# AssemblyAI-Community/MinImagen

Hardware: AMD Instinct MI355X
Metric: denoising-steps/sec (images/sec x T), base 64^2 + SR 64->256 cascade (higher is better)
Workload: dtype f32; 1 GPU; cascade64_256: unet_0 params @64x64 + unet_1 params (lowres_cond) @256x256, T=100/stage, cond_scale=3.0 (2 U-Net evals/step), dynamic thresholding 0.9, fp32 storage / accumulate / softmax / statistics, contractions as 3-term fp16-split (hi*hi + hi*lo + lo*hi) MFMA products; per_gpu_batch=32, global_batch=32, parallelism=dp1

## Files before the change

include/minimagen_hip.h:

```cpp
#ifndef MINIMAGEN_HIP_H
#define MINIMAGEN_HIP_H

#include <stdint.h>

#ifdef __cplusplus
extern "C" {
#endif

#define MI_ABI_VERSION 12

enum mi_status {
    MI_OK = 0,
    MI_ERR_INVALID = -1,
    MI_ERR_LAUNCH = -2,
    MI_ERR_UNSUPPORTED = -3
};

int mi_abi_version(void);
const char* mi_last_error(void);
const char* mi_backend(void);
int mi_struct_size(int which);

typedef struct mi_act {
    const float* data;
// ... 46 lines not shown
int mi_conv_fwd(const mi_conv_params* p, void* stream);
int mi_gn_coef_fwd(const mi_conv_params* p, void* stream);

typedef struct mi_crossembed_params {
    int B, H, W;
    const float* in0; int C0;
    const float* in1; int C1;
    int in1_batch_mod;
    int in0_batch_mod;
    int n_kernels;
    int ksize[3];
    int cout[3];
    const float* w[3];
    const float* bias[3];
    float* out; double* out_stats;
    int out_st;
    int tile_cfg;
    const float* addend;
    const void* w_mfma;
    int w_mfma_exp[3];
} mi_crossembed_params;
int mi_crossembed_fwd(const mi_crossembed_params* p, void* stream);

typedef struct mi_linear {
    const float* w; const float* b; int in, out;
} mi_linear;

typedef struct mi_text_cond_params {
    int B2, B, L, E, cd, tcd, max_len;
    const float* text_embeds;
    const uint8_t* text_mask;
    const uint8_t* keep;
    mi_linear text_to_cond;
    const float* null_text_embed;
    const float* ln_w; const float* ln_b;
    mi_linear h1, h2;
    const float* null_text_hidden;
    const float* norm_w; const float* norm_b;
    float* c_text;
    float* text_hiddens;
} mi_text_cond_params;
int mi_text_cond_fwd(const mi_text_cond_params* p, void* stream);

typedef struct mi_cond_step_params {
    int B2, B, dim, cd, tcd, ntok;
    const int64_t* time;
// ... 302 lines not shown
```

minimagen_amd/_lib.py:

```python
from __future__ import annotations

import ctypes as C
import os

import torch

_HERE = os.path.dirname(os.path.abspath(__file__))
DEFAULT_LIB = os.environ.get("MINIMAGEN_HIP_LIB") or os.path.join(_HERE, "libminimagen_hip.so")

c_float_p = C.c_void_p


class MiAct(C.Structure):
    _fields_ = [("data", C.c_void_p), ("C", C.c_int), ("stats", C.c_void_p), ("nt", C.c_int), ("scale", C.c_float), ("bmod", C.c_int),
                ("st", C.c_int)]


class MiConvParams(C.Structure):
    _fields_ = [
        ("B", C.c_int), ("H", C.c_int), ("W", C.c_int),
        ("in0", MiAct), ("in1", MiAct),
        ("Cout", C.c_int), ("ksize", C.c_int), ("stride", C.c_int), ("up2", C.c_int),
        ("w", C.c_void_p), ("bias", C.c_void_p),
        ("gn_groups", C.c_int), ("gn_gamma", C.c_void_p), ("gn_beta", C.c_void_p), ("gn_eps", C.c_float),
        ("scale_shift", C.c_void_p), ("ss_stride", C.c_int), ("ss_off", C.c_int),
        ("res0", MiAct), ("res1", MiAct), ("res_w", C.c_void_p), ("res_b", C.c_void_p),
        ("out", C.c_void_p), ("out_st", C.c_int), ("out_stats", C.c_void_p), ("tile_cfg", C.c_int),
        ("w_rp", C.c_void_p), ("res_w_rp", C.c_void_p), ("w_rp_exp", C.c_int), ("res_w_rp_exp", C.c_int),
        ("gn_coef", C.c_void_p), ("gn_exps", C.c_void_p),
        ("act_prep", C.c_void_p), ("act_prep_bytes", C.c_longlong),
    ]


class MiCrossEmbedParams(C.Structure):
    _fields_ = [
        ("B", C.c_int), ("H", C.c_int), ("W", C.c_int),
        ("in0", C.c_void_p), ("C0", C.c_int), ("in1", C.c_void_p), ("C1", C.c_int),
        ("in1_batch_mod", C.c_int), ("in0_batch_mod", C.c_int), ("n_kernels", C.c_int),
        ("ksize", C.c_int * 3), ("cout", C.c_int * 3), ("w", C.c_void_p * 3), ("bias", C.c_void_p * 3),
        ("out", C.c_void_p), ("out_stats", C.c_void_p), ("out_st", C.c_int), ("tile_cfg", C.c_int), ("addend", C.c_void_p),
        ("w_mfma", C.c_void_p), ("w_mfma_exp", C.c_int * 3),
    ]


class MiLinear(C.Structure):
    _fields_ = [("w", C.c_void_p), ("b", C.c_void_p), ("in_", C.c_int), ("out", C.c_int)]


class MiTextCondParams(C.Structure):
    _fields_ = [
        ("B2", C.c_int), ("B", C.c_int), ("L", C.c_int), ("E", C.c_int), ("cd", C.c_int), ("tcd", C.c_int), ("max_len", C.c_int),
        ("text_embeds", C.c_void_p), ("text_mask", C.c_void_p), ("keep", C.c_void_p),
        ("text_to_cond", MiLinear), ("null_text_embed", C.c_void_p), ("ln_w", C.c_void_p), ("ln_b", C.c_void_p),
        ("h1", MiLinear), ("h2", MiLinear), ("null_text_hidden", C.c_void_p), ("norm_w", C.c_void_p), ("norm_b", C.c_void_p),
        ("c_text", C.c_void_p), ("text_hiddens", C.c_void_p),
    ]


class MiCondStepParams(C.Structure):
    _fields_ = [
        ("B2", C.c_int), ("B", C.c_int), ("dim", C.c_int), ("cd", C.c_int), ("tcd", C.c_int), ("ntok", C.c_int),
        ("time", C.c_void_p), ("lowres_time", C.c_void_p), ("freq", C.c_void_p),
        ("th", MiLinear), ("tc", MiLinear), ("tt", MiLinear), ("lth", MiLinear), ("ltc", MiLinear), ("ltt", MiLinear),
        ("text_hiddens", C.c_void_p), ("norm_w", C.c_void_p), ("norm_b", C.c_void_p), ("time_mlps", MiLinear),
        ("ss", C.c_void_p), ("c_time", C.c_void_p), ("t_out", C.c_void_p), ("silu_out", C.c_void_p),
    ]

# ... 105 lines not shown
                ("k", C.c_void_p), ("v", C.c_void_p), ("mask", C.c_void_p), ("out", C.c_void_p), ("lse", C.c_void_p), ("dout", C.c_void_p),
                ("dq", C.c_void_p), ("dk", C.c_void_p), ("dv", C.c_void_p), ("work", C.c_void_p), ("work_bytes", C.c_longlong)]


class MiAdamTensor(C.Structure):
    _fields_ = [("p", C.c_void_p), ("g", C.c_void_p), ("m", C.c_void_p), ("v", C.c_void_p), ("n", C.c_longlong)]


class MiAdamParams(C.Structure):
    _fields_ = [("tensors", C.c_void_p), ("chunk_tensor", C.c_void_p), ("chunk_off", C.c_void_p), ("nchunks", C.c_int), ("chunk", C.c_int),
                ("lr", C.c_float), ("beta1", C.c_float), ("beta2", C.c_float), ("eps", C.c_float), ("weight_decay", C.c_float),
                ("bias_correction1", C.c_float), ("bias_correction2", C.c_float), ("one_minus_beta1", C.c_float), ("one_minus_beta2", C.c_float),
                ("grad_scale", C.c_void_p)]


class MiPackConv3Desc(C.Structure):
    _fields_ = [("w", C.c_void_p), ("frag", C.c_void_p), ("generic", C.c_void_p), ("Cout", C.c_int), ("Cin", C.c_int), ("adjoint", C.c_int),
                ("exp", C.c_int), ("cout_pad", C.c_int), ("reserved", C.c_int)]


_STRUCTS = {0: MiAct, 1: MiConvParams, 2: MiCrossEmbedParams, 3: MiLinear, 4: MiTextCondParams, 5: MiCondStepParams,
            6: MiAttnFoldParams, 7: MiCrossAttnParams, 8: MiCfgX0Params, 9: MiQuantileParams, 10: MiPosteriorParams,
            11: MiResizeParams, 12: MiSelfAttnParams, 13: MiChanFFParams, 14: MiFlashAttnParams, 15: MiTokensToNchwParams, 16: MiConvWgradParams, 17: MiBlockBwdParams, 18: MiCrossEmbedWgradParams, 19: MiFoldedAttnParams, 20: MiAdamTensor, 21: MiAdamParams, 22: MiPackConv3Desc,
            23: MiFlashAttnTrainParams, 24: MiSamplerExtParams, 25: MiInpaintParams}

_lib = None
_backend = None


class MinImagenHipError(RuntimeError):
    pass


def _bind(lib):
    lib.mi_abi_version.restype = C.c_int
    lib.mi_last_error.restype = C.c_char_p
    lib.mi_backend.restype = C.c_char_p
    lib.mi_struct_size.argtypes = [C.c_int]
    vp, i32, i64, u64, f32 = C.c_void_p, C.c_int, C.c_int64, C.c_uint64, C.c_float
    for name in ("mi_conv_fwd", "mi_gn_coef_fwd", "mi_crossembed_fwd", "mi_text_cond_fwd", "mi_cond_step_fwd", "mi_attn_fold_rows", "mi_cross_attn_fwd",
                 "mi_cfg_x0_fwd", "mi_quantile_fwd", "mi_posterior_fwd", "mi_resize_fwd", "mi_self_attn_fwd", "mi_chan_ff_fwd",
                 "mi_flash_attn_fwd", "mi_conv_prep_fwd", "mi_tokens_to_nchw_fwd", "mi_conv_wgrad", "mi_block_bwd", "mi_crossembed_wgrad", "mi_folded_attn_fwd", "mi_folded_attn_bwd", "mi_adam_step",
                 "mi_flash_attn_train_fwd", "mi_flash_attn_train_bwd"):
        getattr(lib, name).argtypes = [vp, vp]
        getattr(lib, name).restype = i32
    lib.mi_conv_prep_bytes.argtypes = [i32, i32, i32, i32, i32]
    lib.mi_conv_prep_bytes.restype = C.c_longlong
    lib.mi_flash_kv_prep_bytes.argtypes = [i32, i32]
    lib.mi_flash_kv_prep_bytes.restype = C.c_longlong
    lib.mi_flash_attn_train_workspace.argtypes = [i32, i32, i32, i32, i32, i32]
    lib.mi_flash_attn_train_workspace.restype = C.c_longlong
    lib.mi_step_advance.argtypes = [vp, vp, i32, vp]
    lib.mi_step_advance_by.argtypes = [vp, vp, i32, i32, vp]
    lib.mi_sampler_step_small_fwd.argtypes = [vp, vp, vp, vp]
    lib.mi_sampler_step_small_fwd.restype = i32
    lib.mi_sampler_step_group_fwd.argtypes = [vp, vp, vp, vp, vp]
    lib.mi_sampler_step_group_fwd.restype = i32
    lib.mi_sampler_group_size.argtypes = [i32]
    lib.mi_sampler_group_sync_bytes.argtypes = [i32, i32]
    lib.mi_sampler_group_sync_bytes.restype = C.c_longlong
    lib.mi_step_set.argtypes = [vp, vp, i32, i32, vp]
    lib.mi_posterior_ext_fwd.argtypes = [vp, vp, vp]
    lib.mi_sampler_step_small_ext_fwd.argtypes = [vp, vp, vp, vp, vp]
    lib.mi_sampler_step_group_ext_fwd.argtypes = [vp, vp, vp, vp, vp, vp]
    lib.mi_step_set_mapped.argtypes = [vp, vp, i32, i32, vp, vp]
    lib.mi_step_advance_mapped.argtypes = [vp, vp, i32, vp, vp]
# ... 2 lines not shown
    lib.mi_sampler_step_small_inpaint_fwd.argtypes = [vp, vp, vp, vp, vp, vp]
    lib.mi_sampler_step_group_inpaint_fwd.argtypes = [vp, vp, vp, vp, vp, vp, vp]
    lib.mi_inpaint_blend0_fwd.argtypes = [vp, i32, i32, vp, f32, f32, u64, i32, vp]
    lib.mi_inpaint_prepare_fwd.argtypes = [vp, vp, i32, i32, i32, vp, i32, i32, vp, i32, vp]
    lib.mi_randn_fill.argtypes = [vp, i32, i32, u64, i32, i32, vp]
    lib.mi_finalize_images.argtypes = [vp, vp, i64, i32, vp]
    lib.mi_lowres_augment.argtypes = [vp, vp, vp, i64, f32, f32, i32, vp]
    lib.mi_gemm_f32.argtypes = [vp, vp, vp, vp, vp, i32, i32, i32, i32, vp]
    lib.mi_rmsnorm.argtypes = [vp, vp, vp, i32, i32, f32, vp, vp]
    lib.mi_embed_rows.argtypes = [vp, vp, vp, i32, i32, vp]
    lib.mi_embed_rows_sq.argtypes = [vp, vp, vp, vp, i32, i32, i32, vp]
    lib.mi_gemm_rms_f32.argtypes = [vp, vp, vp, vp, vp, i32, i32, i32, i32, vp, i32, f32, vp, vp]
    lib.mi_t5_attention.argtypes = [vp, vp, vp, vp, i32, i32, i32, vp]
    lib.mi_ln_tokens_fwd.argtypes = [vp, i32, i32, vp, vp, vp, vp]
    lib.mi_ln_rows_fwd.argtypes = [vp, vp, vp, vp, i32, i32, f32, vp]
    lib.mi_graph_begin.argtypes = [vp]
    lib.mi_graph_end.argtypes = [vp, C.POINTER(vp)]
    lib.mi_graph_launch.argtypes = [vp, vp]
    lib.mi_graph_destroy.argtypes = [vp]
    lib.mi_conv_tile_shape.argtypes = [i32, C.POINTER(i32), C.POINTER(i32)]
    lib.mi_conv_stripe_rows.argtypes = [vp]
    lib.mi_conv_stripe_rows.restype = i32
    lib.mi_conv_cout_tile.argtypes = [i32]
    lib.mi_conv_wgrad_workspace.argtypes = [i32, i32, i32]
    lib.mi_conv_wgrad_workspace.restype = C.c_longlong
    lib.mi_crossembed_wgrad_workspace.argtypes = [i32, i32, i32]
    lib.mi_crossembed_wgrad_workspace.restype = C.c_longlong
    lib.mi_chan_stats_fwd.argtypes = [vp, vp, i32, i32, vp]
    lib.mi_layernorm_fwd.argtypes = [vp, vp, vp, vp, vp, i32, i32, C.c_float, vp]
    lib.mi_layernorm_bwd_nwg.argtypes = [i32, i32]
    lib.mi_layernorm_bwd_nwg.restype = i32
    lib.mi_layernorm_bwd.argtypes = [vp, vp, vp, vp, vp, vp, vp, vp, i32, i32, vp]
    lib.mi_pack_conv3_floats.argtypes = [i32, i32, i32, i32, i32]
    lib.mi_pack_conv3_floats.restype = C.c_longlong
    lib.mi_pack_conv3.argtypes = [vp, i32, i32, i32, i32, vp, vp, i32, vp]
    lib.mi_pack_conv3_multi.argtypes = [vp, i32, i32, vp]
    lib.mi_attn_fragment_floats.argtypes = [i32]
    for which, st in _STRUCTS.items():
        n = lib.mi_struct_size(which)
        if n != C.sizeof(st):
            raise MinImagenHipError(f"ABI mismatch: struct {st.__name__} is {n} bytes in the library, {C.sizeof(st)} in the binding")
    return lib


def use_library(path: str):
    global _lib, _backend
# ... 53 lines not shown
```

minimagen_amd/csrc/capi.hip:

```cpp
#include "common.hip.h"
#include <cstdarg>
#include <cstdio>

static thread_local char g_err[512] = "";

void mi_set_error(const char* fmt, ...) {
    va_list ap;
    va_start(ap, fmt);
    vsnprintf(g_err, sizeof(g_err), fmt, ap);
    va_end(ap);
}

int mi_check_launch(const char* what) {
    hipError_t e = hipGetLastError();
    if (e != hipSuccess) {
        mi_set_error("%s: %s", what, hipGetErrorString(e));
        return MI_ERR_LAUNCH;
    }
    return MI_OK;
}

extern "C" int mi_abi_version(void) { return MI_ABI_VERSION; }
extern "C" const char* mi_last_error(void) { return g_err; }
extern "C" const char* mi_backend(void) { return MI_BACKEND_STRING; }
// ... 5 lines not shown
        case 3: return (int)sizeof(mi_linear);
        case 4: return (int)sizeof(mi_text_cond_params);
        case 5: return (int)sizeof(mi_cond_step_params);
        case 6: return (int)sizeof(mi_attn_fold_params);
        case 7: return (int)sizeof(mi_cross_attn_params);
        case 8: return (int)sizeof(mi_cfg_x0_params);
        case 9: return (int)sizeof(mi_quantile_params);
        case 10: return (int)sizeof(mi_posterior_params);
        case 11: return (int)sizeof(mi_resize_params);
        case 12: return (int)sizeof(mi_self_attn_params);
        case 13: return (int)sizeof(mi_chan_ff_params);
        case 14: return (int)sizeof(mi_flash_attn_params);
        case 15: return (int)sizeof(mi_tokens_to_nchw_params);
        case 16: return (int)sizeof(mi_conv_wgrad_params);
        case 17: return (int)sizeof(mi_block_bwd_params);
        case 18: return (int)sizeof(mi_crossembed_wgrad_params);
        case 19: return (int)sizeof(mi_folded_attn_params);
        case 20: return (int)sizeof(mi_adam_tensor);
        case 21: return (int)sizeof(mi_adam_params);
        case 22: return (int)sizeof(mi_pack_conv3_desc);
        case 23: return (int)sizeof(mi_flash_attn_train_params);
        case 24: return (int)sizeof(mi_sampler_ext_params);
        case 25: return (int)sizeof(mi_inpaint_params);
    }
    return -1;
}
```

minimagen_amd/csrc/crossembed.hip:

```cpp
#include "common.hip.h"
#include <type_traits>

namespace {

template <int NT, int TW>
__global__ __launch_bounds__(NT) void crossembed_422_kernel(const mi_crossembed_params p, const float* __restrict__ w3g,
                                                            const float* __restrict__ w7g, const float* __restrict__ w15g) {
    constexpr int TXN = TW / 4, TH = NT / TXN, HALO = 7;
    constexpr int IH = TH + 2 * HALO, IW = TW + 2 * HALO, IWP = (IW + 3) & ~3;
    constexpr int COUT = 8;
    constexpr int STAGE = IH * IWP, RED = 2 * COUT * (NT + 1);
    constexpr int WIN4 = (TW + 16) / 4;
    constexpr int PER4 = (IH * WIN4 + NT - 1) / NT;
    __shared__ __attribute__((aligned(16))) float smem[STAGE > RED ? STAGE : RED];

    const int tid = threadIdx.x;
    const int tiles_x = (p.W + TW - 1) / TW;
    const int tile = blockIdx.x;
    const int oy0 = (tile / tiles_x) * TH, ox0 = (tile % tiles_x) * TW;
    const int b = blockIdx.y;
    const int C0 = p.C0, C1 = p.in1 ? p.C1 : 0, Cin = C0 + C1;
    const int b0 = p.in0_batch_mod > 0 ? b % p.in0_batch_mod : b;
    const int b1 = p.in1_batch_mod > 0 ? b % p.in1_batch_mod : b;
    const int ty = tid / TXN, tx = tid % TXN;
// ... 371 lines not shown
                s += (d0 + d1) + (d2 + d3);
                q2 += fmaf(d0, d0, fmaf(d1, d1, fmaf(d2, d2, d3 * d3)));
            }
        }
        if (p.out_stats) {
#pragma unroll
            for (int o = 1; o <= 4; o <<= 1) { s += __shfl_xor(s, o); q2 += __shfl_xor(q2, o); }
            s += __shfl_xor(s, 16); q2 += __shfl_xor(q2, 16);
            s += __shfl_xor(s, 32); q2 += __shfl_xor(q2, 32);
            if (dy == 0 && lg == 0) {
                mi_stat_acc a; a.c = sh; a.s = s; a.q = q2; a.n = wcnt;
                mi_stat_finish(a, red[wave][2 * (2 * t + co2)], red[wave][2 * (2 * t + co2) + 1]);
            }
        }
    }
    if (p.out_stats) {
        __syncthreads();
        if (tid < 16) p.out_stats[((size_t)(b * 8 + (tid >> 1)) * gridDim.x + tile) * 2 + (tid & 1)] = (red[0][tid] + red[1][tid]) + (red[2][tid] + red[3][tid]);
    }
    CE_TPHASE(3);
    CE_TEND();
}

template <int NT, int TW, int CPT>
__global__ __launch_bounds__(NT) void crossembed_generic_kernel(const mi_crossembed_params p, const int Ctot) {
    constexpr int TH = NT / TW;
    __shared__ double red[2][CPT][NT / 64];
    const int tid = threadIdx.x;
    const int tiles_x = (p.W + TW - 1) / TW;
    const int tile = blockIdx.x;
    const int oy = (tile / tiles_x) * TH + tid / TW, ox = (tile % tiles_x) * TW + tid % TW;
    const int b = blockIdx.y, co_g = blockIdx.z * CPT;
    int ki = 0, co = co_g;
    while (ki < p.n_kernels - 1 && co >= p.cout[ki]) { co -= p.cout[ki]; ++ki; }
    const int K = p.ksize[ki], pad = (K - 1) / 2, CO = p.cout[ki];
    const int C0 = p.C0, C1 = p.in1 ? p.C1 : 0, Cin = C0 + C1;
    const int b0 = p.in0_batch_mod > 0 ? b % p.in0_batch_mod : b;
    const int b1 = p.in1_batch_mod > 0 ? b % p.in1_batch_mod : b;
    float acc[CPT];
#pragma unroll
    for (int j = 0; j < CPT; ++j) acc[j] = 0.0f;
    const bool ok = oy < p.H && ox < p.W;
    if (ok) {
        for (int c = 0; c < Cin; ++c) {
            const float* src = (c < C0) ? p.in0 + (size_t)(b0 * C0 + c) * p.H * p.W
                                        : p.in1 + (size_t)(b1 * C1 + (c - C0)) * p.H * p.W;
// ... 72 lines not shown
            case 0: hipLaunchKernelGGL(HIP_KERNEL_NAME(crossembed_422_kernel<256, 64>), dim3(tiles, p.B), dim3(256), 0, st, p, p.w[0], p.w[1], p.w[2]); break;
            case 1: hipLaunchKernelGGL(HIP_KERNEL_NAME(crossembed_422_kernel<256, 32>), dim3(tiles, p.B), dim3(256), 0, st, p, p.w[0], p.w[1], p.w[2]); break;
            default: hipLaunchKernelGGL(HIP_KERNEL_NAME(crossembed_422_kernel<64, 32>), dim3(tiles, p.B), dim3(64), 0, st, p, p.w[0], p.w[1], p.w[2]); break;
        }
    } else {
        bool oct = true;
        for (int i = 0; i < p.n_kernels; ++i) oct = oct && (p.cout[i] % 8) == 0;
        if (oct) {
            switch (p.tile_cfg) {
                case 0: hipLaunchKernelGGL(HIP_KERNEL_NAME(crossembed_generic_kernel<1024, 64, 8>), dim3(tiles, p.B, Ctot / 8), dim3(1024), 0, st, p, Ctot); break;
                case 1: hipLaunchKernelGGL(HIP_KERNEL_NAME(crossembed_generic_kernel<1024, 32, 8>), dim3(tiles, p.B, Ctot / 8), dim3(1024), 0, st, p, Ctot); break;
                default: hipLaunchKernelGGL(HIP_KERNEL_NAME(crossembed_generic_kernel<256, 32, 8>), dim3(tiles, p.B, Ctot / 8), dim3(256), 0, st, p, Ctot); break;
            }
        } else {
            switch (p.tile_cfg) {
                case 0: hipLaunchKernelGGL(HIP_KERNEL_NAME(crossembed_generic_kernel<1024, 64, 1>), dim3(tiles, p.B, Ctot), dim3(1024), 0, st, p, Ctot); break;
                case 1: hipLaunchKernelGGL(HIP_KERNEL_NAME(crossembed_generic_kernel<1024, 32, 1>), dim3(tiles, p.B, Ctot), dim3(1024), 0, st, p, Ctot); break;
                default: hipLaunchKernelGGL(HIP_KERNEL_NAME(crossembed_generic_kernel<256, 32, 1>), dim3(tiles, p.B, Ctot), dim3(256), 0, st, p, Ctot); break;
            }
        }
    }
    return mi_check_launch("crossembed");
}
```

minimagen_amd/engine.py:

```python
from __future__ import annotations

import ctypes as C
import os
from types import SimpleNamespace
from typing import List, Optional

import torch
from torch import nn

from . import _lib as L
from . import packing as P
from .layers import Attention, CrossAttention, EinopsToAndFrom, Identity, Parallel, ResnetBlock, TransformerBlock

MAX_TEXT_LEN = 256
CONV_SPLIT8 = int(os.environ.get("MINIMAGEN_CONV_SPLIT8", "64"))
CONV_RP = int(os.environ.get("MINIMAGEN_CONV_RP", "2"))
CONV_WIDE_GEMM = os.environ.get("MINIMAGEN_CONV_WIDE_GEMM", "1") != "0"
COND_GEMM = int(os.environ.get("MINIMAGEN_COND_GEMM", "2048"))
FLASH_KV_PREP = os.environ.get("MINIMAGEN_FLASH_KV_PREP", "1") != "0"
CE_MFMA = os.environ.get("MINIMAGEN_CE_MFMA", "1") != "0"
CONV_REVERSE = int(os.environ.get("MINIMAGEN_CONV_REVERSE", "1"))
RP_NTILE = int(os.environ.get("MINIMAGEN_RP_NTILE", "0"))
RP_NTILE_BY = {k: int(os.environ.get("MINIMAGEN_RP_NTILE_" + k, "0")) for k in ("L", "M", "S")}
RP_NTILE_PIPE = {k: int(os.environ.get("MINIMAGEN_RP_NTILE_PIPE_" + k, d)) for k, d in (("L", "0"), ("M", "4"), ("S", "2"))}
CONV_STRIPE = os.environ.get("MINIMAGEN_CONV_STRIPE", "LMS").upper().replace("0", "").replace("1", "LMS")
ST_NBLK = {k: int(os.environ.get("MINIMAGEN_ST_NBLK_" + k, "0")) for k in ("L", "M", "S")}
ST_NBLK_PIPE = {k: int(os.environ.get("MINIMAGEN_ST_NBLK_PIPE_" + k, d)) for k, d in (("L", "0"), ("M", "0"), ("S", "4"))}
WEIGHT_FINGERPRINT = os.environ.get("MINIMAGEN_WEIGHT_FINGERPRINT", "1") != "0"
JT = 17


class Act:
    __slots__ = ("t", "stats", "nt", "C", "H", "W", "batch", "uses", "rev")

    def __init__(self, t, stats, nt, C_, H, W, batch):
        self.t, self.stats, self.nt, self.C, self.H, self.W, self.batch = t, stats, nt, C_, H, W, batch
        self.uses = 0
        self.rev = False

    @property
    def st(self) -> int:
        return 1 if self.t.dtype == torch.bfloat16 else 0

# ... 190 lines not shown
                pk.attn[id(m)] = P.fold_cross_attention(m.to_q.weight, kv_full, m.to_out[0].weight, m.null_kv, m.heads, dh)
        for level in u.downs:
            pre, _, _, _, post = level
            if isinstance(pre, nn.Conv2d):
                pk.conv[id(pre)] = conv_pack(pre)
            if isinstance(post, nn.Conv2d):
                pk.conv[id(post)] = conv_pack(post)
            elif isinstance(post, Parallel):
                w, b = P.fold_parallel_1x1(post.fns[0].weight, post.fns[0].bias, post.fns[1].weight, post.fns[1].bias)
                b = b.contiguous()
                pk.keep.append(b)
                pk.conv[id(post)] = (conv_pack(None, w=w), b)
        for level in u.ups:
            up = level[3]
            if isinstance(up, nn.Sequential):
                pk.conv[id(up[1])] = conv_pack(up[1])
        pk.conv[id(u.final_conv)] = conv_pack(u.final_conv)
        pk.ce_w = [c.weight.detach().permute(1, 2, 3, 0).contiguous() for c in u.init_conv.convs]
        pk.ce_mfma = {}
        cvs = u.init_conv.convs
        if CE_MFMA and [c.kernel_size[0] for c in cvs] == [3, 7, 15] and [c.out_channels for c in cvs] == [4, 2, 2] and u.channels <= 4:
            for chan0 in range(0, cvs[0].in_channels, u.channels):
                pk.ce_mfma[chan0] = P.pack_crossembed_mfma([c.weight for c in cvs], chan0, u.channels)
        self._pack, self._pack_key = pk, key
        return pk

    def packed(self):
        return self._pack if self._pack is not None else self.pack()

    def workspace(self, B: int, B2: int, H: int, W: int, precision: Optional[str] = None, has_text: bool = True, lane: int = 0,
                  pipelined: bool = False) -> Workspace:
        pk = self.packed()
        dev = next(self.unet.parameters()).device
        precision = self.precision if precision is None else precision
        assert precision in ("fp32", "half"), precision
        key = (B, B2, H, W, str(dev), precision, has_text) + ((lane,) if lane else ()) + (("pipe",) if pipelined else ())
        ws = self._ws.get(key)
        if ws is not None:
            return ws
        u = self.unet
        ws = Workspace()
        ws.B, ws.B2, ws.H, ws.W, ws.dev = B, B2, H, W, dev
        ws.pipelined = pipelined
        ws.half = precision == "half"
        f = lambda *shape: torch.zeros(*shape, dtype=torch.float32, device=dev)
        ws.x = f(B, u.channels, H, W)
        ws.lowres = f(B, u.channels, H, W) if u.lowres_cond else None
        ws.times = torch.zeros(B, dtype=torch.int64, device=dev)
# ... 392 lines not shown
        ws.cond_params = cp
        ws.prog_cond = [(lib.mi_cond_step_fwd, cp, "cond_step")]
        if COND_GEMM and pk.R >= COND_GEMM and u.time_cond_dim % 32 == 0:
            cg = L.MiCondStepParams.from_buffer_copy(cp)
            ws.silu_t = self._buf(ws, B2, u.time_cond_dim)
            ws.tm_bias = pk.tm_b.unsqueeze(0).expand(B2, -1).contiguous()
            ws.tensors.append(ws.tm_bias)
            cg.ss, cg.silu_out = 0, L.ptr(ws.silu_t)
            ws.prog_cond = [(lib.mi_cond_step_fwd, cg, "cond_step"),
                            self._call(lib.mi_gemm_f32, "gemm_time_mlps", L.ptr(ws.silu_t), L.ptr(pk.tm_w), 0, L.ptr(ws.tm_bias), L.ptr(ws.ss), B2, pk.R, u.time_cond_dim, 0)]

        cin = u.init_conv.convs[0].in_channels
        assert cin == u.channels * (2 if u.lowres_cond else 1)
        cfg, nt = self._tile_cfg(H, W, B)
        ce_mfma = bool(pk.ce_mfma) and W % 4 == 0
        if ws.store16 and not ce_mfma:
            raise _Store16Unsupported()
        if ce_mfma:
            cfg = 8 if H * W >= 128 * 128 else 9
            th, tw = C.c_int(), C.c_int()
            lib.mi_conv_tile_shape(cfg, C.byref(th), C.byref(tw))
            nt = -(-H // th.value) * -(-W // tw.value)
        ctot = sum(u.init_conv.dim_scales)
        cur = self._new_act(ws, B, ctot, H, W, nt)
        if len(u.init_conv.convs) > 3:
            raise NotImplementedError("CrossEmbedLayer with more than 3 kernel sizes")

        def ce_params(src, chan0, with_bias, out_t, out_stats, addend):
            ce = L.MiCrossEmbedParams()
            ce.B, ce.H, ce.W = B, H, W
            ce.in0, ce.C0 = L.ptr(src), u.channels
            ce.n_kernels = len(u.init_conv.convs)
            for i, cv in enumerate(u.init_conv.convs):
                k, co = cv.kernel_size[0], cv.out_channels
                ce.ksize[i], ce.cout[i] = k, co
                ce.w[i] = L.ptr(pk.ce_w[i]) + 4 * chan0 * k * k * co
                ce.bias[i] = L.ptr(cv.bias) if with_bias else 0
            ce.out, ce.out_stats, ce.tile_cfg, ce.addend = L.ptr(out_t), L.ptr(out_stats), cfg, L.ptr(addend)
            ce.out_st = 1 if ws.store16 else 0
            if ce_mfma:
                tab, exps = pk.ce_mfma[chan0]
                ce.w_mfma, ce.tile_cfg = L.ptr(tab), cfg | (0x400 if ws.half else 0)
                for i in range(3):
                    ce.w_mfma_exp[i] = exps[i]
            return ce

        ws.prog_pre = []
        if u.lowres_cond:
            ws.ce_lr = torch.zeros(B, ctot, H, W, dtype=torch.bfloat16 if ws.store16 else torch.float32, device=ws.dev)
            ws.prog_pre.append((lib.mi_crossembed_fwd, ce_params(ws.lowres, u.channels, False, ws.ce_lr, None, None), "crossembed_lowres"))
            ws.prog.append((lib.mi_crossembed_fwd, ce_params(ws.x, 0, True, cur.t, cur.stats, ws.ce_lr), "crossembed"))
        else:
            ws.prog.append((lib.mi_crossembed_fwd, ce_params(ws.x, 0, True, cur.t, cur.stats, None), "crossembed"))

        hiddens: List[Act] = []
        for pre, init_block, resnet_blocks, attn_block, post in u.downs:
            if isinstance(pre, nn.Conv2d):
                cur = self._emit_conv(ws, pk, cur, None, wpack=pk.conv[id(pre)], bias=pre.bias, Cout=pre.out_channels, ksize=4, stride=2)
            cur = self._emit_resnet(ws, pk, init_block, cur, None)
            for rb in resnet_blocks:
                cur = self._emit_resnet(ws, pk, rb, cur, None)
                hiddens.append(cur)
            if isinstance(attn_block, TransformerBlock):
                cur = self._emit_transformer_block(ws, pk, attn_block, cur)
            hiddens.append(cur)
            if isinstance(post, nn.Conv2d):
                cur = self._emit_conv(ws, pk, cur, None, wpack=pk.conv[id(post)], bias=post.bias, Cout=post.out_channels, ksize=4, stride=2)
            elif isinstance(post, Parallel):
                wp, bsum = pk.conv[id(post)]
                cur = self._emit_conv(ws, pk, cur, None, wpack=wp, bias=bsum, Cout=post.fns[0].out_channels)
        cur = self._emit_resnet(ws, pk, u.mid_block1, cur, None)
        if u.mid_attn is not None:
            cur = self._emit_self_attn(ws, pk, u.mid_attn.fn.fn, cur, want_stats=True)
        cur = self._emit_resnet(ws, pk, u.mid_block2, cur, None)
        for init_block, resnet_blocks, attn_block, upsample in u.ups:
            cur = self._emit_resnet(ws, pk, init_block, cur, hiddens.pop())
            for rb in resnet_blocks:
                cur = self._emit_resnet(ws, pk, rb, cur, hiddens.pop())
            if isinstance(attn_block, TransformerBlock):
                cur = self._emit_transformer_block(ws, pk, attn_block, cur)
# ... 181 lines not shown
```

minimagen_amd/packing.py:

```python
from __future__ import annotations

import math

import torch

LOG2E = 1.4426950408889634


def pack_conv_weight(w: torch.Tensor, cout_tile: int) -> torch.Tensor:
    cout = w.shape[0]
    pad = (cout + cout_tile - 1) // cout_tile * cout_tile
    out = torch.zeros(w.shape[1], w.shape[2], w.shape[3], pad, dtype=torch.float32, device=w.device)
    out[..., :cout] = w.detach().permute(1, 2, 3, 0)
    return out.contiguous()


def fold_parallel_1x1(w3: torch.Tensor, b3, w1: torch.Tensor, b1):
    w = w3.detach().clone()
    w[:, :, 1, 1] += w1.detach()[:, :, 0, 0]
    return w, (b3.detach() + b1.detach())


def fold_cross_attention(to_q, to_kv, to_out, null_kv, heads: int, dim_head: int = 64):
    dev = to_q.device
# ... 147 lines not shown
    return out.reshape(CE_TABLE_ROWS, 256).contiguous().to(ws[0].device), exps


def crossembed_mfma_gather_index(shapes, chan0: int, cin: int):
    idx_w, off = [], 0
    for sh in shapes:
        n = 1
        for d in sh:
            n *= d
        idx_w.append((torch.arange(n, dtype=torch.float64) + (off + 1)).reshape(sh)[:, chan0:chan0 + cin])
        off += n
    tab = _crossembed_toeplitz(idx_w, cin)[:, :, 0]
    idx = tab.round().long() - 1
    idx[idx < 0] = off
    return idx.reshape(-1).contiguous()


def pack_crossembed_mfma_device(ws, idx: torch.Tensor, exps):
    flat = torch.cat([w.detach().reshape(-1) * (2.0 ** e) for w, e in zip(ws, exps)] + [ws[0].new_zeros(1)])
    t = flat[idx].reshape(CE_TABLE_ROWS, 2, 2, 4, 8)
    hi = t.half()
    lo = (t - hi.float()).half()
    return torch.stack((hi, lo), dim=2).reshape(CE_TABLE_ROWS, 256).contiguous()
```

Baseline: 49340 denoising-steps/s.

## Fuse CrossEmbed init conv with first strided downsample via composed weights

Composes the CrossEmbed kernels (3/7/15) and the following 4x4 stride-2 downsample conv into one 18x18 stride-2 convolution with border-dependent weight variants, precomputed on host in double and packed for split-fp16 MFMA. A new kernel computes the downsampled 8-channel output directly, plus GroupNorm stats and the optional lowres addend. This skips writing and re-reading the full-resolution 16-channel CrossEmbed activation and one conv launch per U-Net eval. In exchange the larger composed filter brings extra FLOPs and different rounding from the fp16-split of composed weights.

```diff
diff --git a/include/minimagen_hip.h b/include/minimagen_hip.h
--- a/include/minimagen_hip.h
+++ b/include/minimagen_hip.h
@@ -92,6 +92,26 @@
 } mi_crossembed_params;
 int mi_crossembed_fwd(const mi_crossembed_params* p, void* stream);
 
+typedef struct mi_init_down_params {
+    int B, H, W;
+    const float* in0; int C0;
+    const float* in1; int C1;
+    int in0_batch_mod;
+    int n_kernels;
+    int ksize[3];
+    int cout[3];
+    int Cout;
+    const void* w_tab;
+    int w_exp;
+    const float* bias9;
+    float* out; double* out_stats;
+    int out_st;
+    int tile_cfg;
+    const float* addend;
+} mi_init_down_params;
+int mi_init_down_tiles(int tile_cfg, int H, int W);
+int mi_init_down_fwd(const mi_init_down_params* p, void* stream);
+
 typedef struct mi_linear {
     const float* w; const float* b; int in, out;
 } mi_linear;
diff --git a/minimagen_amd/_lib.py b/minimagen_amd/_lib.py
--- a/minimagen_amd/_lib.py
+++ b/minimagen_amd/_lib.py
@@ -43,6 +43,16 @@
     ]
 
 
+class MiInitDownParams(C.Structure):
+    _fields_ = [
+        ("B", C.c_int), ("H", C.c_int), ("W", C.c_int),
+        ("in0", C.c_void_p), ("C0", C.c_int), ("in1", C.c_void_p), ("C1", C.c_int),
+        ("in0_batch_mod", C.c_int), ("n_kernels", C.c_int), ("ksize", C.c_int * 3), ("cout", C.c_int * 3), ("Cout", C.c_int),
+        ("w_tab", C.c_void_p), ("w_exp", C.c_int), ("bias9", C.c_void_p),
+        ("out", C.c_void_p), ("out_stats", C.c_void_p), ("out_st", C.c_int), ("tile_cfg", C.c_int), ("addend", C.c_void_p),
+    ]
+
+
 class MiLinear(C.Structure):
     _fields_ = [("w", C.c_void_p), ("b", C.c_void_p), ("in_", C.c_int), ("out", C.c_int)]
 
@@ -194,7 +204,7 @@
 _STRUCTS = {0: MiAct, 1: MiConvParams, 2: MiCrossEmbedParams, 3: MiLinear, 4: MiTextCondParams, 5: MiCondStepParams,
             6: MiAttnFoldParams, 7: MiCrossAttnParams, 8: MiCfgX0Params, 9: MiQuantileParams, 10: MiPosteriorParams,
             11: MiResizeParams, 12: MiSelfAttnParams, 13: MiChanFFParams, 14: MiFlashAttnParams, 15: MiTokensToNchwParams, 16: MiConvWgradParams, 17: MiBlockBwdParams, 18: MiCrossEmbedWgradParams, 19: MiFoldedAttnParams, 20: MiAdamTensor, 21: MiAdamParams, 22: MiPackConv3Desc,
-            23: MiFlashAttnTrainParams, 24: MiSamplerExtParams, 25: MiInpaintParams}
+            23: MiFlashAttnTrainParams, 24: MiSamplerExtParams, 25: MiInpaintParams, 26: MiInitDownParams}
 
 _lib = None
 _backend = None
@@ -213,7 +223,7 @@
     for name in ("mi_conv_fwd", "mi_gn_coef_fwd", "mi_crossembed_fwd", "mi_text_cond_fwd", "mi_cond_step_fwd", "mi_attn_fold_rows", "mi_cross_attn_fwd",
                  "mi_cfg_x0_fwd", "mi_quantile_fwd", "mi_posterior_fwd", "mi_resize_fwd", "mi_self_attn_fwd", "mi_chan_ff_fwd",
                  "mi_flash_attn_fwd", "mi_conv_prep_fwd", "mi_tokens_to_nchw_fwd", "mi_conv_wgrad", "mi_block_bwd", "mi_crossembed_wgrad", "mi_folded_attn_fwd", "mi_folded_attn_bwd", "mi_adam_step",
-                 "mi_flash_attn_train_fwd", "mi_flash_attn_train_bwd"):
+                 "mi_flash_attn_train_fwd", "mi_flash_attn_train_bwd", "mi_init_down_fwd"):
         getattr(lib, name).argtypes = [vp, vp]
         getattr(lib, name).restype = i32
     lib.mi_conv_prep_bytes.argtypes = [i32, i32, i32, i32, i32]
@@ -262,6 +272,8 @@
     lib.mi_conv_stripe_rows.argtypes = [vp]
     lib.mi_conv_stripe_rows.restype = i32
     lib.mi_conv_cout_tile.argtypes = [i32]
+    lib.mi_init_down_tiles.argtypes = [i32, i32, i32]
+    lib.mi_init_down_tiles.restype = i32
     lib.mi_conv_wgrad_workspace.argtypes = [i32, i32, i32]
     lib.mi_conv_wgrad_workspace.restype = C.c_longlong
     lib.mi_crossembed_wgrad_workspace.argtypes = [i32, i32, i32]
diff --git a/minimagen_amd/csrc/capi.hip b/minimagen_amd/csrc/capi.hip
--- a/minimagen_amd/csrc/capi.hip
+++ b/minimagen_amd/csrc/capi.hip
@@ -51,6 +51,7 @@
         case 23: return (int)sizeof(mi_flash_attn_train_params);
         case 24: return (int)sizeof(mi_sampler_ext_params);
         case 25: return (int)sizeof(mi_inpaint_params);
+        case 26: return (int)sizeof(mi_init_down_params);
     }
     return -1;
 }
diff --git a/minimagen_amd/csrc/crossembed.hip b/minimagen_amd/csrc/crossembed.hip
--- a/minimagen_amd/csrc/crossembed.hip
+++ b/minimagen_amd/csrc/crossembed.hip
@@ -417,6 +417,229 @@
     CE_TEND();
 }
 
+template <int GX>
+__global__ __launch_bounds__(256, 2) void init_down_mfma_kernel(const mi_init_down_params p, const uint4* __restrict__ wtab, const float* __restrict__ bias9) {
+    constexpr int TWO = 16 * GX;
+    constexpr int IH = 32, PW = 2 * TWO + 24, NW4 = PW / 4, NU = IH * NW4, PER = (NU + 255) / 256;
+    constexpr int ZERO = IH * PW;
+    constexpr int ROWQ = 5 * 2 * 32;
+    __shared__ __attribute__((aligned(16))) uint2 actH[IH * PW + 2];
+    __shared__ __attribute__((aligned(16))) uint2 actL[IH * PW + 2];
+    __shared__ double red[4][16];
+    __shared__ float smax[4];
+    const int tid = threadIdx.x, wave = tid >> 6, lane = tid & 63, lq = lane & 15, lg = lane >> 4;
+    const int H = p.H, W = p.W, HW = H * W, Ho = H >> 1, Wo = W >> 1;
+    const int tiles_x = (Wo + TWO - 1) / TWO, tile = blockIdx.x;
+    const int oy0 = (tile / tiles_x) * 8, ox0 = (tile % tiles_x) * TWO;
+    const int iy0 = 2 * oy0 - 8, ix0 = 2 * ox0 - 8;
+    const int b = blockIdx.y, Cin = p.C0;
+    const int b0 = p.in0_batch_mod > 0 ? b % p.in0_batch_mod : b;
+    const float* src = p.in0 + (size_t)b0 * Cin * HW;
+    const bool vec4 = (Wo & 3) == 0;
+
+    CE_TSTART();
+    float4 raw[PER][4];
+    unsigned inm = 0;
+#pragma unroll
+    for (int u = 0; u < PER; ++u) {
+        const int q = tid + u * 256, iy = q / NW4, xq = q - iy * NW4;
+        const int gy = iy0 + iy, gx = ix0 + 4 * xq;
+        const bool in = q < NU && gy >= 0 && gy < H && gx >= 0 && gx < W;
+        inm |= in ? (1u << u) : 0u;
+        const int off = in ? gy * W + gx : 0;
+#pragma unroll
+        for (int ci = 0; ci < 4; ++ci) raw[u][ci] = ci < Cin ? mi_ldg4(src + (size_t)ci * HW + off) : make_float4(0.f, 0.f, 0.f, 0.f);
+    }
+    const int co = lq >> 1, dy = lq & 1;
+    const int oy = oy0 + 2 * wave + dy;
+    const int vy = oy == 0 ? 0 : (oy == Ho - 1 ? 2 : 1);
+    float4 addv[GX];
+    if (p.addend) {
+#pragma unroll
+        for (int g = 0; g < GX; ++g) {
+            const int ox = ox0 + 16 * g + 4 * lg;
+            const size_t o = ((size_t)(b * 8 + co) * Ho + (oy < Ho ? oy : 0)) * Wo;
+            if (vec4) addv[g] = mi_ldg4(p.addend + o + (oy < Ho && ox < Wo ? ox : 0));
+            else {
+                float a[4];
+#pragma unroll
+                for (int j = 0; j < 4; ++j) a[j] = mi_ldg(p.addend + o + (oy < Ho && ox + j < Wo ? ox + j : 0));
+                addv[g] = make_float4(a[0], a[1], a[2], a[3]);
+            }
+        }
+    }
+    if (tid == 0) { actH[ZERO] = actH[ZERO + 1] = make_uint2(0u, 0u); actL[ZERO] = actL[ZERO + 1] = make_uint2(0u, 0u); }
+    CE_TPHASE(0);
+    float m = 0.0f;
+#pragma unroll
+    for (int u = 0; u < PER; ++u)
+#pragma unroll
+        for (int ci = 0; ci < 4; ++ci) {
+            const float4 v = raw[u][ci];
+            const float a = fmaxf(fmaxf(fabsf(v.x), fabsf(v.y)), fmaxf(fabsf(v.z), fabsf(v.w)));
+            m = ((inm >> u) & 1u) ? fmaxf(m, a) : m;
+        }
+    m = mi_wave_max(m);
+    if (lane == 0) smax[wave] = m;
+    __syncthreads();
+    m = fmaxf(fmaxf(smax[0], smax[1]), fmaxf(smax[2], smax[3]));
+    int ex = 0;
+    {
+        const int be = (int)((__float_as_uint(m) & 0x7fffffffu) >> 23);
+        if (be != 0 && be != 255) ex = 8 - (be - 126);
+    }
+    const float sc = ldexpf(1.0f, ex);
+#pragma unroll
+    for (int u = 0; u < PER; ++u) {
+        const int q = tid + u * 256, iy = q / NW4, xq = q - iy * NW4;
+        if (q >= NU) continue;
+        const bool in = (inm >> u) & 1u;
+        uint2 hh[4], ll[4];
+#pragma unroll
+        for (int j = 0; j < 4; ++j) {
+            float y[4];
+#pragma unroll
+            for (int ci = 0; ci < 4; ++ci) {
+                const float4 v = raw[u][ci];
+                const float x = j == 0 ? v.x : (j == 1 ? v.y : (j == 2 ? v.z : v.w));
+                y[ci] = in ? x * sc : 0.0f;
+            }
+            mi_f16x4 h4, l4;
+            mi_split_f16(y, h4, l4);
+            hh[j] = __builtin_bit_cast(uint2, h4);
+            ll[j] = __builtin_bit_cast(uint2, l4);
+        }
+        const int d = iy * PW + 4 * xq;
+        *reinterpret_cast<uint4*>(&actH[d]) = make_uint4(hh[0].x, hh[0].y, hh[1].x, hh[1].y);
+        *reinterpret_cast<uint4*>(&actH[d + 2]) = make_uint4(hh[2].x, hh[2].y, hh[3].x, hh[3].y);
+        *reinterpret_cast<uint4*>(&actL[d]) = make_uint4(ll[0].x, ll[0].y, ll[1].x, ll[1].y);
+        *reinterpret_cast<uint4*>(&actL[d + 2]) = make_uint4(ll[2].x, ll[2].y, ll[3].x, ll[3].y);
+    }
+    __syncthreads();
+    CE_TPHASE(1);
+
+    const bool hasL = ox0 == 0, hasR = ox0 + TWO >= Wo;
+    const int xr = Wo - 1 - ox0, gR = xr >> 4;
+    f32x4 acc[GX], accL = (f32x4){0.f, 0.f, 0.f, 0.f}, accR = (f32x4){0.f, 0.f, 0.f, 0.f};
+#pragma unroll
+    for (int g = 0; g < GX; ++g) acc[g] = (f32x4){0.f, 0.f, 0.f, 0.f};
+    const uint4* const bbase = wtab + co * 4 + lg;
+    const int a0 = 4 * wave * PW + 2 * lq + 2 * lg;
+    const int aL = lq == 0 ? 4 * wave * PW + 8 + 2 * lg : -1;
+    const int aR = lq == (xr & 15) ? 4 * wave * PW + (W - 2 * ox0) + 2 * lg : -1;
+    struct BRow { uint4 v[5][2]; };
+    struct ARegs { ce_f16x8 h[GX], l[GX]; };
+    auto load_row = [&](int r, BRow& o) {
+        const int ty = r - 2 * dy;
+        const uint4* bp = bbase + ((unsigned)ty < 18u ? vy * 18 + ty : 54) * ROWQ;
+#pragma unroll
+        for (int s = 0; s < 3; ++s) { o.v[s][0] = mi_ldg4u(bp + s * 64); o.v[s][1] = mi_ldg4u(bp + s * 64 + 32); }
+        if (hasL) { o.v[3][0] = mi_ldg4u(bp + 3 * 64); o.v[3][1] = mi_ldg4u(bp + 3 * 64 + 32); }
+        if (hasR) { o.v[4][0] = mi_ldg4u(bp + 4 * 64); o.v[4][1] = mi_ldg4u(bp + 4 * 64 + 32); }
+    };
+    auto load_a = [&](int r, int s, ARegs& a) {
+#pragma unroll
+        for (int g = 0; g < GX; ++g) {
+            const int idx = a0 + r * PW + 32 * g + 8 * s;
+            a.h[g] = __builtin_bit_cast(ce_f16x8, *reinterpret_cast<const uint4*>(&actH[idx]));
+            a.l[g] = __builtin_bit_cast(ce_f16x8, *reinterpret_cast<const uint4*>(&actL[idx]));
+        }
+    };
+    auto load_edge = [&](int idx, ce_f16x8& h, ce_f16x8& l) {
+        h = __builtin_bit_cast(ce_f16x8, *reinterpret_cast<const uint4*>(&actH[idx]));
+        l = __builtin_bit_cast(ce_f16x8, *reinterpret_cast<const uint4*>(&actL[idx]));
+    };
+    auto mma = [&](const ARegs& a, const uint4 (&bv)[2]) {
+        const ce_f16x8 bh = __builtin_bit_cast(ce_f16x8, bv[0]), bl = __builtin_bit_cast(ce_f16x8, bv[1]);
+#pragma unroll
+        for (int g = 0; g < GX; ++g) acc[g] = __builtin_amdgcn_mfma_f32_16x16x32_f16(a.l[g], bh, acc[g], 0, 0, 0);
+#pragma unroll
+        for (int g = 0; g < GX; ++g) acc[g] = __builtin_amdgcn_mfma_f32_16x16x32_f16(a.h[g], bl, acc[g], 0, 0, 0);
+#pragma unroll
+        for (int g = 0; g < GX; ++g) acc[g] = __builtin_amdgcn_mfma_f32_16x16x32_f16(a.h[g], bh, acc[g], 0, 0, 0);
+    };
+    auto mma_edge = [&](f32x4& c, const ce_f16x8& h, const ce_f16x8& l, const uint4 (&bv)[2]) {
+        const ce_f16x8 bh = __builtin_bit_cast(ce_f16x8, bv[0]), bl = __builtin_bit_cast(ce_f16x8, bv[1]);
+        c = __builtin_amdgcn_mfma_f32_16x16x32_f16(l, bh, c, 0, 0, 0);
+        c = __builtin_amdgcn_mfma_f32_16x16x32_f16(h, bl, c, 0, 0, 0);
+        c = __builtin_amdgcn_mfma_f32_16x16x32_f16(h, bh, c, 0, 0, 0);
+    };
+    auto row = [&](int r, int rn, const BRow& o, ARegs& x, ARegs& y) {
+        ce_f16x8 eh[2], el[2];
+        if (hasL) load_edge(aL >= 0 ? aL + r * PW : ZERO, eh[0], el[0]);
+        if (hasR) load_edge(aR >= 0 ? aR + r * PW : ZERO, eh[1], el[1]);
+        load_a(r, 1, y);     mma(x, o.v[0]);
+        load_a(r, 2, x);     mma(y, o.v[1]);
+        load_a(rn, 0, y);    mma(x, o.v[2]);
+        if (hasL) mma_edge(accL, eh[0], el[0], o.v[3]);
+        if (hasR) mma_edge(accR, eh[1], el[1], o.v[4]);
+    };
+    {
+        BRow ba, bb;
+        ARegs ax, ay;
+        load_row(0, ba);
+        load_a(0, 0, ax);
+#pragma unroll 1
+        for (int r = 0; r < 20; r += 2) {
+            load_row(r + 1, bb);
+            row(r, r + 1, ba, ax, ay);
+            load_row(r + 2, ba);
+            row(r + 1, r + 2 < 20 ? r + 2 : 19, bb, ay, ax);
+        }
+    }
+    CE_TPHASE(2);
+
+    const float us = ldexpf(1.0f, -(ex + p.w_exp));
+    float bv[3];
+#pragma unroll
+    for (int vx = 0; vx < 3; ++vx) bv[vx] = bias9 ? mi_ldg(bias9 + (vy * 3 + vx) * 8 + co) : 0.0f;
+    const int wy = Ho - (oy0 + 2 * wave), wx = Wo - ox0;
+    const int wcnt = (wy <= 0 ? 0 : 2) * (wx > TWO ? TWO : wx);
+    float s = 0.0f, q2 = 0.0f, sh = 0.0f;
+#pragma unroll
+    for (int g = 0; g < GX; ++g) {
+        const int ox = ox0 + 16 * g + 4 * lg;
+        float y[4];
+#pragma unroll
+        for (int j = 0; j < 4; ++j) {
+            float a = acc[g][j];
+            if (g == 0) a += hasL ? accL[j] : 0.0f;
+            a += (hasR && g == gR) ? accR[j] : 0.0f;
+            const int X = ox + j;
+            y[j] = fmaf(a, us, X == 0 ? bv[0] : (X == Wo - 1 ? bv[2] : bv[1]));
+        }
+        if (p.addend) { y[0] += addv[g].x; y[1] += addv[g].y; y[2] += addv[g].z; y[3] += addv[g].w; }
+        if (g == 0 && p.out_stats) sh = __shfl(y[0], 2 * co);
+        const size_t o = ((size_t)(b * 8 + co) * Ho + (oy < Ho ? oy : 0)) * Wo;
+        if (vec4) {
+            if (oy < Ho && ox < Wo) mi_stg4(p.out + o + ox, make_float4(y[0], y[1], y[2], y[3]));
+        } else {
+#pragma unroll
+            for (int j = 0; j < 4; ++j)
+                if (oy < Ho && ox + j < Wo) mi_stg(p.out + o + ox + j, y[j]);
+        }
+#pragma unroll
+        for (int j = 0; j < 4; ++j) {
+            const float d = (oy < Ho && ox + j < Wo) ? y[j] - sh : 0.0f;
+            s += d;
+            q2 = fmaf(d, d, q2);
+        }
+    }
+    if (p.out_stats) {
+        s += __shfl_xor(s, 1); q2 += __shfl_xor(q2, 1);
+        s += __shfl_xor(s, 16); q2 += __shfl_xor(q2, 16);
+        s += __shfl_xor(s, 32); q2 += __shfl_xor(q2, 32);
+        if (dy == 0 && lg == 0) {
+            mi_stat_acc a; a.c = sh; a.s = s; a.q = q2; a.n = wcnt;
+            mi_stat_finish(a, red[wave][2 * co], red[wave][2 * co + 1]);
+        }
+        __syncthreads();
+        if (tid < 16) p.out_stats[((size_t)(b * 8 + (tid >> 1)) * gridDim.x + tile) * 2 + (tid & 1)] = (red[0][tid] + red[1][tid]) + (red[2][tid] + red[3][tid]);
+    }
+    CE_TPHASE(3);
+    CE_TEND();
+}
+
 template <int NT, int TW, int CPT>
 __global__ __launch_bounds__(NT) void crossembed_generic_kernel(const mi_crossembed_params p, const int Ctot) {
     constexpr int TH = NT / TW;
@@ -535,3 +758,28 @@
     }
     return mi_check_launch("crossembed");
 }
+
+extern "C" int mi_init_down_tiles(int tile_cfg, int H, int W) {
+    if ((tile_cfg != 0 && tile_cfg != 1) || H < 4 || W < 4 || (H & 1) || (W & 3)) return -1;
+    const int two = tile_cfg == 0 ? 64 : 32;
+    return ((H / 2 + 7) / 8) * ((W / 2 + two - 1) / two);
+}
+
+extern "C" int mi_init_down_fwd(const mi_init_down_params* pp, void* stream) {
+    const mi_init_down_params& p = *pp;
+    hipStream_t st = (hipStream_t)stream;
+    const int tiles = mi_init_down_tiles(p.tile_cfg, p.H, p.W);
+    if (p.B <= 0 || tiles < 0) { mi_set_error("mi_init_down_fwd: B > 0, H and W >= 4, H even, W %% 4 == 0, tile_cfg 0 / 1"); return MI_ERR_INVALID; }
+    if (!p.in0 || !p.w_tab || !p.out) { mi_set_error("mi_init_down_fwd: in0, w_tab and out must be set"); return MI_ERR_INVALID; }
+    int ctot = 0;
+    bool ks_ok = p.n_kernels >= 1 && p.n_kernels <= 3;
+    for (int i = 0; ks_ok && i < p.n_kernels; ++i) { ks_ok = (p.ksize[i] & 1) && p.ksize[i] >= 1 && p.ksize[i] <= 15 && p.cout[i] > 0; ctot += p.cout[i]; }
+    if (!ks_ok || ctot > 16 || p.Cout != 8 || p.C0 < 1 || p.C0 > 4 || p.in1 || p.C1 || p.out_st) {
+        mi_set_error("mi_init_down_fwd: built for a CrossEmbed of <= 3 odd kernels <= 15 with <= 16 channels, 8 Downsample channels, one input of <= 4 channels, fp32 storage");
+        return MI_ERR_UNSUPPORTED;
+    }
+    const uint4* wt = (const uint4*)p.w_tab;
+    if (p.tile_cfg == 0) hipLaunchKernelGGL(HIP_KERNEL_NAME(init_down_mfma_kernel<4>), dim3(tiles, p.B), dim3(256), 0, st, p, wt, p.bias9);
+    else hipLaunchKernelGGL(HIP_KERNEL_NAME(init_down_mfma_kernel<2>), dim3(tiles, p.B), dim3(256), 0, st, p, wt, p.bias9);
+    return mi_check_launch("init_down_mfma");
+}
diff --git a/minimagen_amd/engine.py b/minimagen_amd/engine.py
--- a/minimagen_amd/engine.py
+++ b/minimagen_amd/engine.py
@@ -19,6 +19,7 @@
 COND_GEMM = int(os.environ.get("MINIMAGEN_COND_GEMM", "2048"))
 FLASH_KV_PREP = os.environ.get("MINIMAGEN_FLASH_KV_PREP", "1") != "0"
 CE_MFMA = os.environ.get("MINIMAGEN_CE_MFMA", "1") != "0"
+INIT_DOWN = os.environ.get("MINIMAGEN_INIT_DOWN", "1") != "0"
 CONV_REVERSE = int(os.environ.get("MINIMAGEN_CONV_REVERSE", "1"))
 RP_NTILE = int(os.environ.get("MINIMAGEN_RP_NTILE", "0"))
 RP_NTILE_BY = {k: int(os.environ.get("MINIMAGEN_RP_NTILE_" + k, "0")) for k in ("L", "M", "S")}
@@ -255,8 +256,25 @@
         if CE_MFMA and [c.kernel_size[0] for c in cvs] == [3, 7, 15] and [c.out_channels for c in cvs] == [4, 2, 2] and u.channels <= 4:
             for chan0 in range(0, cvs[0].in_channels, u.channels):
                 pk.ce_mfma[chan0] = P.pack_crossembed_mfma([c.weight for c in cvs], chan0, u.channels)
+        pk.init_down = {}
+        pre0 = u.downs[0][0]
+        pk.init_down_ok = INIT_DOWN and CE_MFMA and isinstance(pre0, nn.Conv2d) and pre0.kernel_size == (4, 4) and pre0.stride == (2, 2) \
+            and pre0.padding == (1, 1) and pre0.out_channels == 8 and len(cvs) <= 3 and all(c.kernel_size[0] % 2 == 1 and c.kernel_size[0] <= 15 for c in cvs) \
+            and sum(c.out_channels for c in cvs) <= 16 and u.channels <= 4 and not u.init_conv_to_final_conv_residual
         self._pack, self._pack_key = pk, key
         return pk
+
+    def _init_down_tables(self, pk):
+        if not pk.init_down:
+            u = self.unet
+            cvs, pre0 = u.init_conv.convs, u.downs[0][0]
+            dev = pre0.weight.device
+            for chan0 in range(0, cvs[0].in_channels, u.channels):
+                x_half = chan0 == 0
+                w9, b9 = P.compose_init_down([c.weight for c in cvs], [c.bias for c in cvs] if x_half else None, pre0.weight, pre0.bias, chan0, u.channels)
+                tab, exp, b32 = P.pack_init_down_mfma(w9, b9)
+                pk.init_down[chan0] = (tab.to(dev), exp, b32.to(dev) if x_half else None)
+        return pk.init_down
 
     def packed(self):
         return self._pack if self._pack is not None else self.pack()
@@ -695,9 +713,9 @@
             lib.mi_conv_tile_shape(cfg, C.byref(th), C.byref(tw))
             nt = -(-H // th.value) * -(-W // tw.value)
         ctot = sum(u.init_conv.dim_scales)
-        cur = self._new_act(ws, B, ctot, H, W, nt)
         if len(u.init_conv.convs) > 3:
             raise NotImplementedError("CrossEmbedLayer with more than 3 kernel sizes")
+        init_down = pk.init_down_ok and not ws.half and not ws.store16 and H >= 4 and W >= 4 and H % 2 == 0 and W % 4 == 0
 
         def ce_params(src, chan0, with_bias, out_t, out_stats, addend):
             ce = L.MiCrossEmbedParams()
@@ -718,17 +736,40 @@
                     ce.w_mfma_exp[i] = exps[i]
             return ce
 
+        def id_params(src, chan0, out_t, out_stats, addend, id_cfg):
+            q = L.MiInitDownParams()
+            q.B, q.H, q.W = B, H, W
+            q.in0, q.C0 = L.ptr(src), u.channels
+            q.n_kernels = len(u.init_conv.convs)
+            for i, cv in enumerate(u.init_conv.convs):
+                q.ksize[i], q.cout[i] = cv.kernel_size[0], cv.out_channels
+            tab, q.w_exp, b9 = pk.init_down[chan0]
+            q.Cout, q.w_tab, q.bias9 = 8, L.ptr(tab), L.ptr(b9)
+            q.out, q.out_stats, q.tile_cfg, q.addend = L.ptr(out_t), L.ptr(out_stats), id_cfg, L.ptr(addend)
+            return q
+
         ws.prog_pre = []
-        if u.lowres_cond:
-            ws.ce_lr = torch.zeros(B, ctot, H, W, dtype=torch.bfloat16 if ws.store16 else torch.float32, device=ws.dev)
-            ws.prog_pre.append((lib.mi_crossembed_fwd, ce_params(ws.lowres, u.channels, False, ws.ce_lr, None, None), "crossembed_lowres"))
-            ws.prog.append((lib.mi_crossembed_fwd, ce_params(ws.x, 0, True, cur.t, cur.stats, ws.ce_lr), "crossembed"))
+        if init_down:
+            self._init_down_tables(pk)
+            id_cfg = 0 if W // 2 >= 64 else 1
+            cur = self._new_act(ws, B, 8, H // 2, W // 2, lib.mi_init_down_tiles(id_cfg, H, W))
+            fn = lib.mi_init_down_fwd
+            if u.lowres_cond:
+                ws.ce_lr = torch.zeros(B, 8, H // 2, W // 2, dtype=torch.float32, device=ws.dev)
+                ws.prog_pre.append((fn, id_params(ws.lowres, u.channels, ws.ce_lr, None, None, id_cfg), "crossembed_lowres"))
+            ws.prog.append((fn, id_params(ws.x, 0, cur.t, cur.stats, ws.ce_lr if u.lowres_cond else None, id_cfg), "crossembed"))
         else:
-            ws.prog.append((lib.mi_crossembed_fwd, ce_params(ws.x, 0, True, cur.t, cur.stats, None), "crossembed"))
+            cur = self._new_act(ws, B, ctot, H, W, nt)
+            if u.lowres_cond:
+                ws.ce_lr = torch.zeros(B, ctot, H, W, dtype=torch.bfloat16 if ws.store16 else torch.float32, device=ws.dev)
+                ws.prog_pre.append((lib.mi_crossembed_fwd, ce_params(ws.lowres, u.channels, False, ws.ce_lr, None, None), "crossembed_lowres"))
+                ws.prog.append((lib.mi_crossembed_fwd, ce_params(ws.x, 0, True, cur.t, cur.stats, ws.ce_lr), "crossembed"))
+            else:
+                ws.prog.append((lib.mi_crossembed_fwd, ce_params(ws.x, 0, True, cur.t, cur.stats, None), "crossembed"))
 
         hiddens: List[Act] = []
-        for pre, init_block, resnet_blocks, attn_block, post in u.downs:
-            if isinstance(pre, nn.Conv2d):
+        for level, (pre, init_block, resnet_blocks, attn_block, post) in enumerate(u.downs):
+            if isinstance(pre, nn.Conv2d) and not (init_down and level == 0):
                 cur = self._emit_conv(ws, pk, cur, None, wpack=pk.conv[id(pre)], bias=pre.bias, Cout=pre.out_channels, ksize=4, stride=2)
             cur = self._emit_resnet(ws, pk, init_block, cur, None)
             for rb in resnet_blocks:
diff --git a/minimagen_amd/packing.py b/minimagen_amd/packing.py
--- a/minimagen_amd/packing.py
+++ b/minimagen_amd/packing.py
@@ -193,3 +193,57 @@
     hi = t.half()
     lo = (t - hi.float()).half()
     return torch.stack((hi, lo), dim=2).reshape(CE_TABLE_ROWS, 256).contiguous()
+
+
+ID_TAPS = 18
+ID_ROWS = 3 * ID_TAPS + 1
+ID_STEPS = 5
+
+
+def compose_init_down(ce_ws, ce_bs, wd, bd, chan0: int, cin: int):
+    ks = [w.shape[-1] for w in ce_ws]
+    assert all(k % 2 == 1 and k <= 15 for k in ks) and tuple(wd.shape[2:]) == (4, 4)
+    m_tot = sum(w.shape[0] for w in ce_ws)
+    assert wd.shape[1] == m_tot
+    wc = torch.zeros(m_tot, cin, 15, 15, dtype=torch.float64)
+    m0 = 0
+    for w, k in zip(ce_ws, ks):
+        o = (15 - k) // 2
+        wc[m0:m0 + w.shape[0], :, o:o + k, o:o + k] = w.detach().double().cpu()[:, chan0:chan0 + cin]
+        m0 += w.shape[0]
+    wdd = wd.detach().double().cpu()
+    co = wdd.shape[0]
+    with_bias = ce_bs is not None
+    bc = torch.cat([b.detach().double().cpu() for b in ce_bs]) if with_bias else torch.zeros(m_tot, dtype=torch.float64)
+    taps = ((1, 2, 3), (0, 1, 2, 3), (0, 1, 2))
+    w9 = torch.zeros(3, 3, co, cin, ID_TAPS, ID_TAPS, dtype=torch.float64)
+    b9 = torch.zeros(3, 3, co, dtype=torch.float64)
+    for vy in range(3):
+        for vx in range(3):
+            for a in taps[vy]:
+                for b in taps[vx]:
+                    w9[vy, vx, :, :, a:a + 15, b:b + 15] += torch.einsum('om,mcyx->ocyx', wdd[:, :, a, b], wc)
+                    b9[vy, vx] += wdd[:, :, a, b] @ bc
+            if with_bias and bd is not None:
+                b9[vy, vx] += bd.detach().double().cpu()
+    return w9, b9
+
+
+def pack_init_down_mfma(w9: torch.Tensor, b9: torch.Tensor):
+    co, cin = w9.shape[2], w9.shape[3]
+    assert co == 8 and cin <= 4 and tuple(w9.shape[4:]) == (ID_TAPS, ID_TAPS)
+    wp = torch.zeros(3, 3, co, 4, ID_TAPS, 24, dtype=torch.float64)
+    wp[:, :, :, :cin, :, :ID_TAPS] = w9
+    exp = rp_weight_exponent(float(wp.abs().max()))
+    wp = wp * (2.0 ** exp)
+    tab = torch.zeros(ID_ROWS, ID_STEPS, co, 4, 2, 4, dtype=torch.float64)
+    f = lambda t, n: t.reshape(3, co, 4, ID_TAPS, n, 4, 2).permute(0, 3, 4, 1, 5, 6, 2)
+    main = tab[:3 * ID_TAPS].reshape(3, ID_TAPS, ID_STEPS, co, 4, 2, 4)
+    main[:, :, 0:3] = f(wp[:, 1], 3)
+    main[:, :, 3] = f((wp[:, 0] - wp[:, 1])[..., 8:16], 1)[:, :, 0]
+    main[:, :, 4] = f((wp[:, 2] - wp[:, 1])[..., 2:10], 1)[:, :, 0]
+    t = tab.reshape(ID_ROWS, ID_STEPS, co, 4, 8)
+    hi = t.float().half()
+    lo = (t - hi.double()).float().half()
+    out = torch.stack((hi, lo), dim=2)
+    return out.reshape(ID_ROWS, -1).contiguous(), exp, b9.float().contiguous()
```

Result: faster. 50440 denoising-steps/s (median of 6 runs) (+2.2%).
